# Sara-H-dev/Semantic_Segmentation_Of_StyleGAN2_Artifacts

Hardware: AMD Instinct MI355X
Metric: training images/sec at 1024^2 bs=8 per GPU (MS-UNet Swin-T, fwd+DynamicLoss+bwd+AdamW) (higher is better)
Workload: dtype bf16; 1 GPU; 1xMI355X 1024x1024 bs=8 Swin-T MS-UNet train step; model=MS-UNet swin_t, global_batch=8, world_size=1, img_size=1024, parallelism=dp1, grad_allreduce=f32, dead_branches=executed (no grad), step_execution=eager, params=42881040

## Files before the change

include/msunet_hip.h:

```cpp
#ifndef MSUNET_HIP_H
#define MSUNET_HIP_H

#ifdef __cplusplus
extern "C" {
#endif

int msu_layernorm_fwd(int dtype, int mode, const void* x, const void* b, const float* bscale,
                      long rows_per_sample, void* s_out, const float* gamma, const float* beta,
                      void* y, float* mean, float* rstd, long rows, int C, int H, int W, int Cin,
                      float eps, void* stream);
int msu_layernorm_bwd(int dtype, int mode, const void* dy, const void* x, const void* dres,
                      const float* gamma, const float* mean, const float* rstd, void* dx,
                      void* db, const float* bscale, long rows_per_sample, float* part,
                      int nparts, float* dgamma, float* dbeta, long rows, int C, int H, int W,
                      int Cin, int accumulate, void* stream);
int msu_layernorm_bwd3(int dtype, int mode, const void* dy, const void* x, const void* dres,
                       const void* dres2, const void* dres3, const float* gamma, const float* mean,
                       const float* rstd, void* dx, void* db, const float* bscale, long rows_per_sample,
                       float* part, int nparts, float* dgamma, float* dbeta, long rows, int C, int H, int W,
                       int Cin, int accumulate, void* stream);
int msu_ln_part_blocks(long rows, int C);
int msu_colsum_batch(int nseg, const float* const* part, const long* stride, const int* nparts, const int* n,
                     float* const* out, int accumulate, void* stream);
int msu_tail_reduce_mode(int mode);
// ... 27 lines not shown
                     void* stream);
int msu_win_attn_bwd2(int dtype, const void* qkv, const float* qkv_bias, const float* table,
                      const void* dout, void* dqkv, float* dtable, float* dqkv_bias_pad,
                      float* workspace, int B, int H, int W, int C, int nh, int shift,
                      float p_drop, unsigned long long seed, const unsigned long long* seed_dev, const void* keep,
                      void* stream, void* param_stream);
int msu_win_attn_bwd_tail(int dtype, float* workspace, float* dtable, float* dqkv_bias_pad, int B, int H, int W,
                          int C, int nh, void* stream);
int msu_win_attn_bwd_tail2(int dtype, float* workspace, float* dtable, float* dqkv_bias_pad, int B, int H, int W,
                           int C, int nh, int accumulate, void* stream);

int msu_conv3x3_fwd(int dtype, int in_mode, const void* X, const void* Wt, const float* bias,
                    void* Y, int B, int H, int W, int Cin, int Cout, void* stream);
int msu_conv3x3_fwd2(int dtype, int in_mode, const void* X, const void* Wt, const float* bias,
                     void* Y, void* Y2, int B, int H, int W, int Cin, int Cout, void* stream);
int msu_conv3x3_dgrad(int dtype, int out_mode, const void* dY, const void* Wflip, const void* S,
                      void* dX, int B, int H, int W, int Cin, int Cout, void* stream);
int msu_conv_mode(int mode);
long msu_conv3x3_wgrad_workspace(int nchunk, int Cin, int Cout, int dtype, int unused);
int msu_conv3x3_wgrad(int dtype, int in_mode, const void* X, const void* dY, float* dW, float* db,
                      float* workspace, void* unused, int nchunk, int B, int H, int W, int Cin,
                      int Cout, void* stream);
int msu_conv3x3_wgrad2(int dtype, int in_mode, const void* X, const void* dY, float* dW, float* db,
                       float* workspace, int nchunk, int B, int H, int W, int Cin, int Cout, int accumulate,
                       void* stream);

int msu_win_attn_qkv_supported(int C, int nh);
int msu_win_attn_qkv_fwd(int dtype, const void* x, const void* w_qkv, const float* b_qkv, const float* table,
                         void* out, void* qkv_out, void* keep, float* workspace, int B, int H, int W, int C, int nh,
                         int shift, float p_drop, unsigned long long seed, const unsigned long long* seed_dev,
// ... 99 lines not shown
```

semantic_segmentation_of_stylegan2_artifacts_amd/_lib.py:

```python
import ctypes
import os

from . import switches

_HERE = os.path.dirname(os.path.abspath(__file__))
LIB_PATH = switches.get("MSU_LIB_OVERRIDE") or os.path.join(_HERE, "libmsunet_hip.so")

P = ctypes.c_void_p
I = ctypes.c_int
L = ctypes.c_long
F = ctypes.c_float
D = ctypes.c_double
U64 = ctypes.c_ulonglong

SIGNATURES = {
    "msu_ln_part_blocks": (I, [L, I]),
    "msu_layernorm_fwd": (I, [I, I, P, P, P, L, P, P, P, P, P, P, L, I, I, I, I, F, P]),
    "msu_layernorm_bwd": (I, [I, I, P, P, P, P, P, P, P, P, P, L, P, I, P, P, L, I, I, I, I, I, P]),
    "msu_layernorm_bwd3": (I, [I, I, P, P, P, P, P, P, P, P, P, P, P, L, P, I, P, P, L, I, I, I, I, I, P]),
    "msu_reduce_rows": (I, [P, I, I, L, P, I, P]),
    "msu_tail_reduce_mode": (I, [I]),
    "msu_conv_mode": (I, [I]),
    "msu_head_fwd": (I, [I, P, P, P, P, P, P, P, L, I, F, P]),
    "msu_head_bwd": (I, [I, P, P, P, P, P, P, P, P, P, I, P, P, P, L, I, P]),
# ... 23 lines not shown
    "msu_dynloss_fwd2": (I, [I, P, P, I, L, F, F, F, P, I, P, P, P, P]),
    "msu_dynloss_fwd3": (I, [I, P, P, I, L, F, F, F, P, I, P, P, P, P, P]),
    "msu_dynloss_bwd2": (I, [I, P, P, P, P, P, I, L, F, F, F, P, P]),
    "msu_adamw": (I, [P, P, P, P, L, F, F, F, F, F, I, P, P, P]),
    "msu_nonfinite": (I, [P, L, P, P]),
    "msu_nonfinite2": (I, [P, L, P, L, P, P]),
    "msu_adamw_dev": (I, [P, P, P, P, L, P, D, D, D, D, P, P, P]),
    "msu_adamw_dev2": (I, [P, P, P, P, L, P, D, D, D, D, P, P, P, I, I, P]),
    "msu_step_advance": (I, [P, P, P]),
    "msu_cast": (I, [I, P, P, L, P]),
    "msu_colsum_batch": (I, [I, P, P, P, P, P, I, P]),
    "msu_conv3x3_weight": (I, [I, P, P, I, I, I, P]),
    "msu_transpose16_multi": (I, [P, P, P, I, I, P]),
    "msu_conv3x3_fwd": (I, [I, I, P, P, P, P, I, I, I, I, I, P]),
    "msu_conv3x3_fwd2": (I, [I, I, P, P, P, P, P, I, I, I, I, I, P]),
    "msu_conv3x3_dgrad": (I, [I, I, P, P, P, P, I, I, I, I, I, P]),
    "msu_conv3x3_wgrad_workspace": (L, [I, I, I, I, I]),
    "msu_conv3x3_wgrad": (I, [I, I, P, P, P, P, P, P, I, I, I, I, I, I, P]),
    "msu_conv3x3_wgrad2": (I, [I, I, P, P, P, P, P, I, I, I, I, I, I, I, P]),
    "msu_wgrad_splits": (I, [L, I, I]),
    "msu_wgrad_workspace": (L, [L, I, I]),
    "msu_linear_wgrad": (I, [I, P, P, P, P, P, L, I, I, I, P]),
    "msu_linear_wgrad_ld": (I, [I, P, P, P, L, P, P, L, I, I, I, P]),
    "msu_linear_bwd_supported": (I, [L, I, I]),
    "msu_linear_bwd_workspace": (L, [L, I, I]),
    "msu_linear_bwd": (I, [I, P, P, P, P, P, P, P, P, L, I, I, I, P]),
    "msu_tok_gemm_supported": (I, [L, I, I]),
    "msu_tok_gemm_supported_epi": (I, [L, I, I, I]),
    "msu_tok_gemm": (I, [I, P, P, I, P, P, P, P, P, L, I, I, I, P]),
    "msu_tok_gemm_plan": (I, [L, I, I, P]),
# ... 13 lines not shown
_lib = None


class HipLibraryError(RuntimeError):
    pass


def lib():
    global _lib
    if _lib is not None:
        return _lib
    if not os.path.exists(LIB_PATH):
        raise HipLibraryError(
            f"{LIB_PATH} not found: build it with "
            "`python -m semantic_segmentation_of_stylegan2_artifacts_amd.build` (no CPU fallback)")
    h = ctypes.CDLL(LIB_PATH)
    for name, (res, args) in SIGNATURES.items():
        fn = getattr(h, name)
        fn.restype = res
        fn.argtypes = args
    h.msu_nt_gemm_mode((1 if switches.on("MSU_NT_PP") else 0) | (16 if switches.on("MSU_NT_DYN") else 0))
    h.msu_tail_reduce_mode(1 if switches.on("MSU_TAIL") else 0)
    h.msu_conv_mode(1 if switches.on("MSU_CONV_DYN") else 0)
    _lib = h
    return _lib


def plan_nt(M, N):
    v = lib().msu_nt_gemm_plan(M, N)
    return (v % 1000000) // 1000, v % 1000, v >= 1000000


def call(name, *args):
    rc = getattr(lib(), name)(*args)
    if rc != 0:
        raise HipLibraryError(f"{name} failed with code {rc}")
# ... 2 lines not shown
```

semantic_segmentation_of_stylegan2_artifacts_amd/csrc/conv3x3.h:

```cpp
#pragma once
#include <cstdlib>
#include <utility>

#include "common.h"
#include "mfma_frag.h"
#include "reduce.h"

#ifndef MSU_EXP
#define MSU_EXP 0
#endif

namespace {

constexpr int TW = 16;

struct ConvGeom {
  int B, H, W;
  int Cin, CinP;
  int Cout;
  int PS;
  int PSW;
  int PSD;
};

// ... 423 lines not shown
          }
        }
    }
  }
}

constexpr int V3_HALO_TAP = 1;
constexpr int SPRE = 12;
constexpr bool SP_AT7 = (MSU_EXP & 1024) != 0;

MSU_DEV int swz(int p) { return (p >> 2) & 3; }
template <bool M16> MSU_DEV int swzv(int p) { return M16 ? (p >> 1) & 3 : (p >> 2) & 3; }

MSU_DEV constexpr int halo_part_lo(int t, int nhc) { return (t - 1) * nhc / 7; }

template <typename T, bool IN_D2S, bool OUT_D2S, bool OUT_GGRAD, bool BIAS, bool DUAL, bool SPREAD, bool M16>
__global__ void __launch_bounds__(512) conv3x3_v3_kernel(const bf16_t* __restrict__ X,
                                                         const bf16_t* __restrict__ Wt,
                                                         const float* __restrict__ bias,
                                                         const bf16_t* __restrict__ S,
                                                         bf16_t* __restrict__ Y, bf16_t* __restrict__ Y2,
                                                         ConvGeom g, int ntiles, int* __restrict__ tq) {
  constexpr int C = 96, CH = 12, NW = 8, MT = 2, TH = NW * MT, TWV = 32, HWD = TWV + 2;
  constexpr int HPIX = (TH + 2) * HWD;
  (void)HPIX;
  constexpr int NTHR = 64 * NW;
  constexpr int PSTEP = NTHR / CH;
  constexpr int NHC = (HPIX + PSTEP - 1) / PSTEP;
  constexpr int WIMG = C * C;
  constexpr int WINS = WIMG * 2 / 1024;
  constexpr int WPER = (WINS + NW - 1) / NW;
  static_assert(WINS * 1024 == WIMG * 2, "weight image in whole DMA instructions");

  extern __shared__ __attribute__((aligned(16))) unsigned char smem_raw[];
  bf16_t* sX = reinterpret_cast<bf16_t*>(smem_raw);
  bf16_t* sW = sX + HPIX * C;
  float* sB = reinterpret_cast<float*>(sW + 2 * WIMG);
  int* sQ = reinterpret_cast<int*>(sB + C);
  const int tid = threadIdx.x, lane = tid & 63;
  const int wave = __builtin_amdgcn_readfirstlane(tid >> 6);
  const int tiles_x = (g.W + TWV - 1) / TWV, tiles_y = (g.H + TH - 1) / TH;
  constexpr int EST = MT * 6 * (DUAL ? 2 : 1);
  const int per_img = tiles_x * tiles_y;

  auto coords = [&](int tile, int& b, int& y0, int& x0) {
    b = tile / per_img;
    const int r = tile - b * per_img;
    y0 = (r / tiles_x) * TH;
    x0 = (r - (r / tiles_x) * tiles_x) * TWV;
  };
  u32x4 hr[NHC];
  auto load_halo = [&](int tile, auto C0, auto C1) {
    constexpr int c0 = decltype(C0)::value, c1 = decltype(C1)::value;
    int b, y0, x0;
    coords(tile, b, y0, x0);
    const int t = opaque(tid);
    const bool hact = t < PSTEP * CH;
// ... 48 lines not shown

  auto finish = [&]() { tq_finish(tq); };
  auto read_q = [&]() -> int {
    uint32_t v = ds_b32_untracked<0>(lds_u32(sQ));
    lds_wait_tie<0>(v);
    return __builtin_amdgcn_readfirstlane((int)v) + (int)gridDim.x;
  };
  int tile = blockIdx.x;
  if (tile >= ntiles) {
    finish();
    return;
  }
  if (tq != nullptr && tid == 0) sQ[0] = tq_claim(tq, 0);
  if constexpr (BIAS) {
    if (tid < C) sB[tid] = bias[tid];
  }
  load_halo(tile, IC<0>{}, IC<NHC>{});
  store_halo();
  dma_w(0, 0);
  __syncthreads();
  int next = tq != nullptr ? read_q() : tile + (int)gridDim.x;
  int wbuf = 0;
  bool w1_early = false, st_full = false;

  const int xl = lane & 31, h = lane >> 5;
  auto koff = [&](int sw, int odd) { return ((2 * odd + h) ^ sw) << 3; };
  const int wsw = swz(xl);
  const int wk0 = xl * C + koff(wsw, 0), wk1 = xl * C + koff(wsw, 1);
  const int l15 = lane & 15, g4 = lane >> 4;
  const int wk16 = l15 * C + ((g4 ^ swzv<true>(l15)) << 3);
// ... 203 lines not shown
      }
      wbuf ^= 1;
    }, std::make_integer_sequence<int, 9>{});
    auto epi_start = [&]() __attribute__((always_inline)) {
      if constexpr (OUT_GGRAD) {
        wait_vmcnt<0>();
#pragma unroll
        for (int m = 0; m < MT; ++m)
#pragma unroll
          for (int n = 0; n < (M16 ? 2 : 3); ++n)
#pragma unroll
            for (int pp = 0; pp < (M16 ? 3 : 2); ++pp) vreg_pin(sp[m][n][pp]);
      }
      w1_early = next < ntiles;
      st_full = w1_early && x0 + TWV <= g.W && y0 + TH <= g.H;
      if (w1_early) dma_w(1, wbuf ^ 1);
    };

    if constexpr (M16) {
      const int cofs = 16 * (g4 & 1) + 8 * (g4 >> 1);
      float4 bq[3][2];
      if constexpr (BIAS) {
#pragma unroll
        for (int q = 0; q < 3; ++q) {
          bq[q][0] = *reinterpret_cast<const float4*>(sB + 32 * q + cofs);
          bq[q][1] = *reinterpret_cast<const float4*>(sB + 32 * q + cofs + 4);
        }
      }
      epi_start();
#pragma unroll
      for (int pt = 0; pt < 2; ++pt) {
        const int px = x0 + 16 * pt + l15;
        if (px >= g.W) continue;
#pragma unroll
        for (int q = 0; q < 3; ++q) {
          float bv[8] = {0.f, 0.f, 0.f, 0.f, 0.f, 0.f, 0.f, 0.f};
          if constexpr (BIAS) {
            const float4 t0 = bq[q][0], t1 = bq[q][1];
            bv[0] = t0.x; bv[1] = t0.y; bv[2] = t0.z; bv[3] = t0.w;
            bv[4] = t1.x; bv[5] = t1.y; bv[6] = t1.z; bv[7] = t1.w;
          }
#pragma unroll
          for (int m = 0; m < MT; ++m) {
            const int y = y0 + 2 * wave + m;
// ... 9 lines not shown
            if constexpr (OUT_GGRAD) {
              const u32x4 t = sp[m][pt][q];
#pragma unroll
              for (int i = 0; i < 4; ++i) {
                v[2 * i] *= gelu_grad_fast(Fmt16<T>::lo(t[i]));
                v[2 * i + 1] *= gelu_grad_fast(Fmt16<T>::hi(t[i]));
              }
            }
            const u32x4 pk = {pack2<T>(v[0], v[1]), pack2<T>(v[2], v[3]), pack2<T>(v[4], v[5]), pack2<T>(v[6], v[7])};
            const int off = pix_off32<OUT_D2S>(b, y, px, g.H, g.W, C) + 32 * q + cofs;
            if constexpr (MSU_EXP & 64) if (v[0] != 1.2345e-30f) continue;
            *reinterpret_cast<u32x4*>(Y + off) = pk;
            if constexpr (DUAL) *reinterpret_cast<u32x4*>(Y2 + off) = gelu8<T>(pk);
          }
        }
      }
    } else {
    float4 bq[3][2][2];
    if constexpr (BIAS) {
#pragma unroll
      for (int n = 0; n < 3; ++n)
#pragma unroll
        for (int pp = 0; pp < 2; ++pp) {
          const int co = 32 * n + 16 * pp + 8 * h;
          bq[n][pp][0] = *reinterpret_cast<const float4*>(sB + co);
          bq[n][pp][1] = *reinterpret_cast<const float4*>(sB + co + 4);
        }
    }
    epi_start();
    if (xo < g.W) {
// ... 369 lines not shown
  static_assert(lds <= 160 * 1024, "LDS");
  auto kern = conv3x3_v2_kernel<T, NCT, KS, NW, MT, WDB, IN_D2S, IN_GELU, OUT_D2S, OUT_GGRAD, BIAS, DUAL>;
  static bool attr_set = false;
  if (!attr_set) {
    (void)hipFuncSetAttribute((const void*)kern, hipFuncAttributeMaxDynamicSharedMemorySize, (int)lds);
    attr_set = true;
  }
  const long ntiles = (long)g.B * ((g.W + 31) / 32) * ((g.H + TH - 1) / TH);
  if (ntiles == 0) return 0;
  if ((long)g.B * g.H * g.W * (g.Cin > g.Cout ? g.Cin : g.Cout) >= (1L << 31)) return -2;
  const int grid = (int)(ntiles < num_cus() ? ntiles : num_cus());
  hipLaunchKernelGGL(kern, dim3(grid), dim3(64 * NW), lds, st, X, Wt, bias, S, Y, Y2, g, (int)ntiles);
  return MSU_CHECK_LAUNCH();
}

template <typename T, bool IN_D2S, bool OUT_D2S, bool OUT_GGRAD, bool BIAS, bool DUAL, bool SPREAD, bool M16>
int launch_v3s(const ConvGeom& g, const bf16_t* X, const bf16_t* Wt, const float* bias, const bf16_t* S, bf16_t* Y,
               bf16_t* Y2, hipStream_t st) {
  constexpr size_t lds = sizeof(bf16_t) * ((size_t)18 * 34 * 96 + 2 * 96 * 96) + 96 * sizeof(float) + 16;
  static_assert(lds <= 160 * 1024, "LDS");
  auto kern = conv3x3_v3_kernel<T, IN_D2S, OUT_D2S, OUT_GGRAD, BIAS, DUAL, SPREAD, M16>;
  static bool attr_set = false;
  if (!attr_set) {
    (void)hipFuncSetAttribute((const void*)kern, hipFuncAttributeMaxDynamicSharedMemorySize, (int)lds);
    attr_set = true;
  }
  const long ntiles = (long)g.B * ((g.W + 31) / 32) * ((g.H + 15) / 16);
  if (ntiles == 0) return 0;
  if ((long)g.B * g.H * g.W * 96 >= (1L << 31)) return -2;
  const int grid = (int)(ntiles < num_cus() ? ntiles : num_cus());
  hipLaunchKernelGGL(kern, dim3(grid), dim3(512), lds, st, X, Wt, bias, S, Y, Y2, g, (int)ntiles,
                     g_conv_dyn ? tile_queue(st) : nullptr);
  return MSU_CHECK_LAUNCH();
}

template <typename T, bool IN_D2S, bool OUT_D2S, bool OUT_GGRAD, bool BIAS, bool DUAL>
int launch_v3(const ConvGeom& g, const bf16_t* X, const bf16_t* Wt, const float* bias, const bf16_t* S, bf16_t* Y,
              bf16_t* Y2, hipStream_t st) {
  if constexpr (!OUT_GGRAD || (MSU_EXP & 2048) != 0)
    return launch_v3s<T, IN_D2S, OUT_D2S, OUT_GGRAD, BIAS, DUAL, true, true>(g, X, Wt, bias, S, Y, Y2, st);
  return launch_v3s<T, IN_D2S, OUT_D2S, OUT_GGRAD, BIAS, DUAL, true, false>(g, X, Wt, bias, S, Y, Y2, st);
}

template <typename T, bool IN_D2S, bool IN_GELU, bool OUT_D2S, bool OUT_GGRAD, bool BIAS, bool DUAL = false>
int conv_nt(const ConvGeom& g, const void* X, const void* Wt, const float* bias, const void* S,
            void* Y, void* Y2, hipStream_t st) {
  const T* x = (const T*)X; const T* w = (const T*)Wt; const T* s = (const T*)S; T* y = (T*)Y; T* y2 = (T*)Y2;
  if constexpr (sizeof(T) == 2 && !IN_GELU) {
// ... 76 lines not shown
```

semantic_segmentation_of_stylegan2_artifacts_amd/csrc/conv3x3.hip:

```cpp
#include "conv3x3.h"

extern "C" {

int msu_conv3x3_fwd2(int dtype, int in_mode, const void* X, const void* Wt, const float* bias,
                     void* Y, void* Y2, int B, int H, int W, int Cin, int Cout, void* stream) {
  if (Cout % 16 || Cin % 8 || Cout > 128 || Cin > 128) return -2;
  if ((in_mode & 2) && (H % 4 || W % 4)) return -2;
  if (Y2 && (in_mode & 1)) return -2;
  const ConvGeom g = make_geom(B, H, W, Cin, Cout, msu_is16(dtype) ? 2 : 4);
  hipStream_t st = (hipStream_t)stream;
  if (bias == nullptr) return -2;
#define MSU_FWD(T, D2S, GL, DU) return conv_nt<T, D2S, GL, false, false, true, DU>(g, X, Wt, bias, nullptr, Y, Y2, st)
#define MSU_FWD_ALL(T)                              \
  switch ((in_mode & 3) | (Y2 ? 4 : 0)) {           \
    case 0: MSU_FWD(T, false, false, false);        \
    case 1: MSU_FWD(T, false, true, false);         \
    case 2: MSU_FWD(T, true, false, false);         \
    case 3: MSU_FWD(T, true, true, false);          \
    case 4: MSU_FWD(T, false, false, true);         \
    case 6: MSU_FWD(T, true, false, true);          \
  }
  if (dtype == MSU_BF16) {
    MSU_FWD_ALL(bf16_t)
  } else if (dtype == MSU_F16) {
    MSU_FWD_ALL(f16_t)
  } else {
    MSU_FWD_ALL(float)
  }
#undef MSU_FWD_ALL
#undef MSU_FWD
  return -3;
}

int msu_conv3x3_fwd(int dtype, int in_mode, const void* X, const void* Wt, const float* bias,
                    void* Y, int B, int H, int W, int Cin, int Cout, void* stream) {
  return msu_conv3x3_fwd2(dtype, in_mode, X, Wt, bias, Y, nullptr, B, H, W, Cin, Cout, stream);
}

int msu_conv3x3_dgrad(int dtype, int out_mode, const void* dY, const void* Wflip, const void* S,
                      void* dX, int B, int H, int W, int Cin, int Cout, void* stream) {
  if (Cout % 16 || Cin % 16 || Cout > 128 || Cin > 128) return -2;
  if ((out_mode & 2) && (H % 4 || W % 4)) return -2;
  const ConvGeom g = make_geom(B, H, W, Cout, Cin, msu_is16(dtype) ? 2 : 4);
  hipStream_t st = (hipStream_t)stream;
#define MSU_DG(T, D2S, GG) return conv_nt<T, false, false, D2S, GG, false>(g, dY, Wflip, nullptr, S, dX, nullptr, st)
  if (dtype == MSU_BF16) {
    switch (out_mode & 3) {
      case 1: MSU_DG(bf16_t, false, true);
      case 3: MSU_DG(bf16_t, true, true);
    }
  } else if (dtype == MSU_F16) {
    switch (out_mode & 3) {
      case 1: MSU_DG(f16_t, false, true);
// ... 20 lines not shown
```

semantic_segmentation_of_stylegan2_artifacts_amd/network/model_parts.py:

```python
import math
import random

import torch
import torch.nn as nn
import torch.nn.functional as F

from .. import ops


def _trunc_normal_(t, std=0.02):
    return nn.init.trunc_normal_(t, std=std)


def _to_2tuple(v):
    return tuple(v) if isinstance(v, (tuple, list)) else (v, v)


def _relative_position_index(ws):
    coords = torch.stack(torch.meshgrid(torch.arange(ws), torch.arange(ws), indexing="ij"))
    flat = coords.flatten(1)
    rel = (flat[:, :, None] - flat[:, None, :]).permute(1, 2, 0).contiguous()
    rel[:, :, 0] += ws - 1
    rel[:, :, 1] += ws - 1
    rel[:, :, 0] *= 2 * ws - 1
# ... 289 lines not shown

    def __init__(self, input_resolution, dim, dim_scale=4, norm_layer=nn.LayerNorm):
        super().__init__()
        self.input_resolution = input_resolution
        self.dim = dim
        self.dim_scale = dim_scale
        if dim_scale != 4:
            raise ValueError("FinalPatchExpand_X4_V2 is a x4 expand")
        self.expand = nn.Linear(dim, 16 * dim, bias=False)
        self.act = nn.GELU()
        self.output_dim = dim
        self.refine1 = nn.Conv2d(dim, dim, kernel_size=3, padding=1, bias=True)
        self.refine2 = nn.Conv2d(dim, dim, kernel_size=3, padding=1, bias=True)
        self.norm = norm_layer(self.output_dim)

    def pre_norm(self, x):
        H, W = self.input_resolution
        B, L, C = x.shape
        assert L == H * W, "input feature has wrong size"
        e, a0 = ops.linear_gelu(x, self.expand.weight)
        e, a0 = e.view(B, H, W, 16 * C), a0.view(B, H, W, 16 * C)
        z1, a1 = ops.refine_conv_act(e, a0, self.refine1.weight, self.refine1.bias, True, (4 * H, 4 * W), dual=True)
        return ops.refine_conv_act(z1, a1, self.refine2.weight, self.refine2.bias, False, (4 * H, 4 * W))

    def forward(self, x):
        z2 = self.pre_norm(x)
        B = z2.shape[0]
        y = ops.layer_norm(z2, self.norm.weight, self.norm.bias, self.norm.eps)
        return y.reshape(B, -1, self.output_dim)


class BasicLayer_up(nn.Module):

    def __init__(self, dim, input_resolution, depth, num_heads, window_size, mlp_ratio=4.0,
                 qkv_bias=True, qk_scale=None, drop=0.0, attn_drop=0.0, drop_path=0.0,
                 norm_layer=nn.LayerNorm, upsample=None, use_checkpoint=False):
        super().__init__()
        self.dim = dim
# ... 192 lines not shown
            else:
                x = _skip_fuse(self.concat_back_dim[k], x, xd[3 - k], keys[3 - k] if keys else 0)
                x = layer_up(x)
        return ops.layer_norm(x, self.norm_up.weight, self.norm_up.bias, self.norm_up.eps)

    def up_x4(self, x):
        H, W = self.patches_resolution
        if x.dim() == 4:
            B, H, W, C = x.shape
            x = x.reshape(B, H * W, C)
        else:
            B, L, C = x.shape
            assert L == H * W, "input features has wrong size"
        if self.final_upsample != "expand_first":
            return x
        z2 = self.up.pre_norm(x)
        if self.num_classes == 1:
            return ops.head_norm_output(z2, self.up.norm.weight, self.up.norm.bias, self.output.weight,
                                        self.up.norm.eps)
        y = ops.layer_norm(z2, self.up.norm.weight, self.up.norm.bias, self.up.norm.eps)
        return ops.linear(y, self.output.weight.reshape(self.num_classes, -1)).permute(0, 3, 1, 2)

    def forward(self, x):
        x, xd, xk = self._forward_features(x)
        x = self.forward_up_features(x, xd, xk)
        return self.up_x4(x)

    def freeze_encoder(self, freeze=True):
        for p in self.patch_embed.parameters():
            p.requires_grad = not freeze
# ... 16 lines not shown
```

semantic_segmentation_of_stylegan2_artifacts_amd/ops.py:

```python
import contextlib
import ctypes
import functools

import torch

from . import _lib, switches

_DT = {torch.float32: 0, torch.bfloat16: 1, torch.float16: 2}
_LOW = (torch.bfloat16, torch.float16)


def _dt(t):
    try:
        return _DT[t.dtype]
    except KeyError:
        raise TypeError(f"unsupported activation dtype {t.dtype} (float32 / bfloat16 / float16)") from None


def _need_cuda(*ts):
    for t in ts:
        if t is not None and not t.is_cuda:
            raise RuntimeError("msunet HIP ops need tensors on a HIP device (no CPU fallback)")


# ... 1301 lines not shown

def _head_fake(z, gamma, beta, w, eps):
    B, H, W, C = z.shape
    rows = B * H * W
    return (z.new_empty(B, 1, H, W, dtype=torch.float32), z.new_empty(rows, dtype=torch.float32),
            z.new_empty(rows, dtype=torch.float32))


def _head_setup(ctx, inputs, output):
    z, gamma, beta, w, eps = inputs
    ctx.save_for_backward(z.contiguous(), gamma, beta, w, output[1], output[2])
    ctx.params = (gamma, beta, w)
    ctx.set_materialize_grads(False)


def _head_backward(ctx, dlogit, _dm, _dr):
    z, gamma, beta, w, mean, rstd = ctx.saved_tensors
    if dlogit is None:
        return None, None, None, None, None
    B, H, W, C = z.shape
    rows = B * H * W
    dlogit = _f32(dlogit)
    dz = torch.empty_like(z)
    direct = _direct(*ctx.params)
    if direct:
        dg, db, dw = (p.grad for p in ctx.params)
    else:
        dg, db, dw = torch.empty(3, C, device=z.device, dtype=torch.float32)
    n, part = _ln_parts(rows, C, z.device)
    _lib.call("msu_head_bwd2", _dt(z), _p(dlogit), _p(z), _p(gamma), _p(beta), _p(w), _p(mean),
              _p(rstd), _p(dz), _p(part), n, _p(dg), _p(db), _p(dw), rows, C, int(direct), _s(z))
    if direct:
        _notify(*ctx.params)
        return dz, None, None, None, None
    return dz, dg, db, dw.view(w.shape), None


_head = _define("head_norm_output",
                "(Tensor z, Tensor gamma, Tensor beta, Tensor w, float eps) -> (Tensor, Tensor, Tensor)",
                _head_impl, _head_fake, _head_setup, _head_backward)


def head_norm_output(z, gamma, beta, out_weight, eps=1e-5):
    if out_weight.shape[0] != 1:
        raise ValueError("fused head supports num_classes == 1")
    w = _f32(out_weight).contiguous()
    return _head(_as(z, act_dtype()), _f32(gamma), _f32(beta), w, float(eps))[0]


_CONV_WGRAD_BLOCKS = int(switches.get("MSU_CONV_WGRAD_BLOCKS"))
# ... 96 lines not shown

def _refine_act_fake(x, a, weight, bias, d2s, H, W, dual):
    z = a.new_empty(a.shape[0], H, W, weight.shape[0])
    return z, (torch.empty_like(z) if dual else z.new_empty(0))


def _refine_act_setup(ctx, inputs, output):
    x, a, weight, bias, d2s, H, W, dual = inputs
    ctx.save_for_backward(x, a.contiguous(), weight)
    ctx.params = (weight, bias)
    ctx.cfg = (d2s, H, W)
    ctx.mark_non_differentiable(output[1])
    ctx.set_materialize_grads(False)


def _refine_act_backward(ctx, dz, _dz2):
    x, a, weight = ctx.saved_tensors
    d2s, H, W = ctx.cfg
    if dz is None:
        return (None,) * 8
    Cout, Cin = weight.shape[0], weight.shape[1]
    B = a.shape[0]
    dz = _as(dz, a.dtype)
    dx = None
    if ctx.needs_input_grad[0]:
        wf = _conv_weight(weight, a.dtype, 1)
        dx = torch.empty_like(x)
        _lib.call("msu_conv3x3_dgrad", _dt(a), 1 | (2 if d2s else 0), _p(dz), _p(wf), _p(x), _p(dx),
                  B, H, W, Cin, Cout, _s(a))
    dw, db = _conv_wgrad_param(a, dz, 2 if d2s else 0, B, H, W, Cin, Cout, *ctx.params)
    return dx, None, dw, db, None, None, None, None


_refine_conv_act = _define(
    "refine_conv_act",
    "(Tensor x, Tensor a, Tensor weight, Tensor bias, bool d2s, int H, int W, bool dual) -> (Tensor, Tensor)",
    _refine_act_impl, _refine_act_fake, _refine_act_setup, _refine_act_backward)


def refine_conv_act(x, a, weight, bias, d2s, out_hw, dual=False):
    dt = act_dtype()
    H, W = out_hw
    z, z2 = _refine_conv_act(_as(x, dt), _as(a, dt), _f32(weight), _f32(bias), bool(d2s), int(H), int(W),
                             bool(dual))
    return (z, z2) if dual else z


_zero_bias_cache = {}


def _zero_bias(N, device):
    key = (N, str(device))
    z = _zero_bias_cache.get(key)
    if z is None:
        z = torch.zeros(N, device=device, dtype=torch.float32)
        if not torch.cuda.is_current_stream_capturing():
            _zero_bias_cache[key] = z
    return z


# ... 253 lines not shown
```

semantic_segmentation_of_stylegan2_artifacts_amd/switches.py:

```python
import os
import warnings

SWITCHES = {
    "MSU_LIB_OVERRIDE": ("", "path of another libmsunet_hip.so (tools/build_exp.sh ablation builds)",
                         "DESIGN 4c"),
    "MSU_WGRAD_SIDE": ("1", "0: every weight gradient on the main stream (determinism bisection)",
                       "DESIGN 4b, 7 (side stream +1.6 %)"),
    "MSU_ATTN_QKV": ("1", "0: the unfused stage-0 qkv Linear + window attention + proj",
                     "DESIGN 4d (r04c: +0.8 %)"),
    "MSU_GEMM_ROUTE": ("", "force a GEMM route: lib (hipBLASLt) / tok / nt",
                       "DESIGN 7 (r03c: hand-written +2.7 % over hipBLASLt)"),
    "MSU_NT_PP": ("0", "1: the ping-pong NT GEMM (gemm_pp.h) where it tiles exactly, else the persistent one",
                  "DESIGN 7 (r05g: 0.72-0.98x of the persistent kernel; no-store ablation 1.07-1.66x)"),
    "MSU_LINBWD": ("1", "0: stage-0 Linear backward as input-gradient GEMM + side-stream weight gradient",
                   "DESIGN 7 (r03af: one-pass +1.4 %)"),
    "MSU_CONV_SIDE": ("1", "0: the refine-conv weight gradients on the main stream",
                      "DESIGN 7 (r04s: side +0.2 %)"),
    "MSU_TAIL": ("1", "0: LayerNorm parameter-gradient partials summed by a colsum launch, not in the kernel",
                 "DESIGN 7 (r05i: +0.5 %, host -4 ms/step)"),
    "MSU_ATTN_AUX": ("1", "0: each attention backward rebuilds its relative-bias image instead of reusing the "
                     "forward's workspace", "DESIGN 7 (r05az)"),
    "MSU_MLP_INFER": ("1", "0: no-grad stage-0 MLPs on the token-GEMM pair instead of the fused kernel",
                      "DESIGN 7 (r05am: +1.3 %)"),
    "MSU_MLP_LN": ("1", "0: no-grad stage-0 blocks run norm2's residual-add LayerNorm as its own kernel before the "
                   "fused MLP", "DESIGN 7 (r05at)"),
    "MSU_MLP_TRAIN": ("1", "0: training stage-0 MLPs on the token-GEMM pair (H and GELU(H) stored) instead of "
                      "the fused kernel storing H only", "DESIGN 7 (r05ao)"),
    "MSU_LN_DEFER": ("1", "0: each LayerNorm backward sums its parameter-gradient partials itself (in-kernel "
                     "tail) instead of one batched reduction per width", "DESIGN 7 (r06)"),
    "MSU_NT_DYN": ("0", "1: the NT GEMM's two-stage kernel claims tiles from a per-XCD device queue (measured "
                   "-0.3 % step, 1.8 % slower standalone: r06q/r06r)", "DESIGN 7 (r06)"),
    "MSU_CONV_DYN": ("1", "0: the refine-conv kernel's static tile schedule (blockIdx.x + k * gridDim.x) instead "
                     "of the device tile queue", "DESIGN 7 (r06)"),
    "MSU_CONV_WGRAD_BLOCKS": ("256", "persistent workgroups of the refine-conv weight gradient (one per CU by "
                              "default; fewer leave CUs to the main stream)", "DESIGN 7 (r04ac, r06)"),
    "MSU_MLP_S1": ("1", "0: the stage-1 training MLPs on the GEMM pair (H and GELU(H) stored) instead of the "
                   "fused kernel streaming its weights through an LDS ring", "DESIGN 7 (r06)"),
    "MSU_RES_HANDOFF": ("1", "0: a stage's first Swin block sums its input's two gradients (norm1 LayerNorm, norm2 "
                        "residual) with an ATen add instead of inside the LayerNorm backward", "DESIGN 7 (r06)"),
    "MSU_GRAPH": ("auto", "HIP-graph replay of the step: 1 / 0 / auto (replay when launch-bound)",
                  "DESIGN 4b (512^2: 401 vs 249-307 img/s)"),
    "MSU_GRAPH_SIDE": ("0", "1: fork the side stream into the captured graph (nondeterministic on ROCm 7.2)",
                       "DESIGN 4b (r03h)"),
}

VALUES = {name: os.environ.get(name, d[0]) for name, d in SWITCHES.items()}


def get(name):
    return VALUES[name]


def on(name):
    return VALUES[name] != "0"
# ... 15 lines not shown
```

Before: 178.8 images/s.

## Fuse decoder head LayerNorm and 1x1 output conv into refine2 conv epilogue

Adds a HEAD variant of the refine conv kernel whose epilogue computes the per-pixel LayerNorm statistics and the dot product with gamma*w_out, writing the logit, mean and rstd directly. When gradients are needed it still stores z for the backward pass. This removes the separate head forward kernel and its re-read of the full-resolution 96-channel activation. It also removes the unused NT_DYN switch. The cost is a longer epilogue with extra cross-lane reductions and more register pressure in the conv kernel.

Measured after the change: 179.5 images/s, median of 6. No clear change (+0.4%).

```diff
diff --git a/include/msunet_hip.h b/include/msunet_hip.h
--- a/include/msunet_hip.h
+++ b/include/msunet_hip.h
@@ -65,6 +65,10 @@
                     void* Y, int B, int H, int W, int Cin, int Cout, void* stream);
 int msu_conv3x3_fwd2(int dtype, int in_mode, const void* X, const void* Wt, const float* bias,
                      void* Y, void* Y2, int B, int H, int W, int Cin, int Cout, void* stream);
+int msu_conv3x3_fwd_head(int dtype, int mode, const void* A, const void* Wt, const float* bias, void* Z,
+                         const float* gamma, const float* beta, const float* w_out, float* logit,
+                         float* mean, float* rstd, int B, int H, int W, int Cin, int Cout, float eps,
+                         void* stream);
 int msu_conv3x3_dgrad(int dtype, int out_mode, const void* dY, const void* Wflip, const void* S,
                       void* dX, int B, int H, int W, int Cin, int Cout, void* stream);
 int msu_conv_mode(int mode);
diff --git a/semantic_segmentation_of_stylegan2_artifacts_amd/_lib.py b/semantic_segmentation_of_stylegan2_artifacts_amd/_lib.py
--- a/semantic_segmentation_of_stylegan2_artifacts_amd/_lib.py
+++ b/semantic_segmentation_of_stylegan2_artifacts_amd/_lib.py
@@ -61,6 +61,7 @@
     "msu_transpose16_multi": (I, [P, P, P, I, I, P]),
     "msu_conv3x3_fwd": (I, [I, I, P, P, P, P, I, I, I, I, I, P]),
     "msu_conv3x3_fwd2": (I, [I, I, P, P, P, P, P, I, I, I, I, I, P]),
+    "msu_conv3x3_fwd_head": (I, [I, I, P, P, P, P, P, P, P, P, P, P, I, I, I, I, I, F, P]),
     "msu_conv3x3_dgrad": (I, [I, I, P, P, P, P, I, I, I, I, I, P]),
     "msu_conv3x3_wgrad_workspace": (L, [I, I, I, I, I]),
     "msu_conv3x3_wgrad": (I, [I, I, P, P, P, P, P, P, I, I, I, I, I, I, P]),
@@ -104,12 +105,13 @@
         raise HipLibraryError(
             f"{LIB_PATH} not found: build it with "
             "`python -m semantic_segmentation_of_stylegan2_artifacts_amd.build` (no CPU fallback)")
+    import torch
     h = ctypes.CDLL(LIB_PATH)
     for name, (res, args) in SIGNATURES.items():
         fn = getattr(h, name)
         fn.restype = res
         fn.argtypes = args
-    h.msu_nt_gemm_mode((1 if switches.on("MSU_NT_PP") else 0) | (16 if switches.on("MSU_NT_DYN") else 0))
+    h.msu_nt_gemm_mode(1 if switches.on("MSU_NT_PP") else 0)
     h.msu_tail_reduce_mode(1 if switches.on("MSU_TAIL") else 0)
     h.msu_conv_mode(1 if switches.on("MSU_CONV_DYN") else 0)
     _lib = h
diff --git a/semantic_segmentation_of_stylegan2_artifacts_amd/csrc/conv3x3.h b/semantic_segmentation_of_stylegan2_artifacts_amd/csrc/conv3x3.h
--- a/semantic_segmentation_of_stylegan2_artifacts_amd/csrc/conv3x3.h
+++ b/semantic_segmentation_of_stylegan2_artifacts_amd/csrc/conv3x3.h
@@ -461,13 +461,40 @@
 
 MSU_DEV constexpr int halo_part_lo(int t, int nhc) { return (t - 1) * nhc / 7; }
 
-template <typename T, bool IN_D2S, bool OUT_D2S, bool OUT_GGRAD, bool BIAS, bool DUAL, bool SPREAD, bool M16>
+struct ConvHead {
+  const float* gamma;
+  const float* beta;
+  const float* w;
+  float* logit;
+  float* mean;
+  float* rstd;
+  float eps;
+};
+
+MSU_DEV float quad_sum(float s) {
+  auto r = __builtin_amdgcn_permlane16_swap(__float_as_uint(s), __float_as_uint(s), false, false);
+  s = __uint_as_float(r[0]) + __uint_as_float(r[1]);
+  r = __builtin_amdgcn_permlane32_swap(__float_as_uint(s), __float_as_uint(s), false, false);
+  return __uint_as_float(r[0]) + __uint_as_float(r[1]);
+}
+
+template <int OFF>
+MSU_DEV f32x4 ds_b128_untracked(uint32_t addr) {
+  f32x4 v;
+  asm volatile("ds_read_b128 %0, %1 offset:%2" : "=v"(v) : "v"(addr), "i"(OFF));
+  return v;
+}
+
+template <typename T, bool IN_D2S, bool OUT_D2S, bool OUT_GGRAD, bool BIAS, bool DUAL, bool SPREAD, bool M16,
+          bool HEAD = false>
 __global__ void __launch_bounds__(512) conv3x3_v3_kernel(const bf16_t* __restrict__ X,
                                                          const bf16_t* __restrict__ Wt,
                                                          const float* __restrict__ bias,
                                                          const bf16_t* __restrict__ S,
                                                          bf16_t* __restrict__ Y, bf16_t* __restrict__ Y2,
-                                                         ConvGeom g, int ntiles, int* __restrict__ tq) {
+                                                         ConvGeom g, int ntiles, int* __restrict__ tq,
+                                                         ConvHead hd) {
+  static_assert(!HEAD || (M16 && BIAS && !OUT_D2S && !OUT_GGRAD && !DUAL), "HEAD: the refine2 forward form");
   constexpr int C = 96, CH = 12, NW = 8, MT = 2, TH = NW * MT, TWV = 32, HWD = TWV + 2;
   constexpr int HPIX = (TH + 2) * HWD;
   (void)HPIX;
@@ -484,10 +511,11 @@
   bf16_t* sW = sX + HPIX * C;
   float* sB = reinterpret_cast<float*>(sW + 2 * WIMG);
   int* sQ = reinterpret_cast<int*>(sB + C);
+  float* sG = reinterpret_cast<float*>(sQ + 4);
   const int tid = threadIdx.x, lane = tid & 63;
   const int wave = __builtin_amdgcn_readfirstlane(tid >> 6);
   const int tiles_x = (g.W + TWV - 1) / TWV, tiles_y = (g.H + TH - 1) / TH;
-  constexpr int EST = MT * 6 * (DUAL ? 2 : 1);
+  constexpr int EST = MT * 6 * (DUAL ? 2 : 1) + (HEAD ? MT * 2 * 3 : 0);
   const int per_img = tiles_x * tiles_y;
 
   auto coords = [&](int tile, int& b, int& y0, int& x0) {
@@ -566,6 +594,21 @@
   if (tq != nullptr && tid == 0) sQ[0] = tq_claim(tq, 0);
   if constexpr (BIAS) {
     if (tid < C) sB[tid] = bias[tid];
+  }
+  float bwsum = 0.f;
+  if constexpr (HEAD) {
+    if (tid < C) sG[tid] = hd.gamma[tid] * hd.w[tid];
+    float bp[4];
+#pragma unroll
+    for (int l = 0; l < 4; ++l) {
+      bp[l] = 0.f;
+#pragma unroll
+      for (int k = 0; k < 3; ++k)
+#pragma unroll
+        for (int e = 0; e < 8; ++e) bp[l] += hd.beta[(l + 4 * k) * 8 + e] * hd.w[(l + 4 * k) * 8 + e];
+    }
+    bwsum = (bp[0] + bp[2]) + (bp[1] + bp[3]);
+    bwsum = __uint_as_float(__builtin_amdgcn_readfirstlane(__float_as_uint(bwsum)));
   }
   load_halo(tile, IC<0>{}, IC<NHC>{});
   store_halo();
@@ -799,13 +842,16 @@
       }
       w1_early = next < ntiles;
       st_full = w1_early && x0 + TWV <= g.W && y0 + TH <= g.H;
+      if constexpr (HEAD) st_full = st_full && Y != nullptr;
       if (w1_early) dma_w(1, wbuf ^ 1);
     };
 
     if constexpr (M16) {
-      const int cofs = 16 * (g4 & 1) + 8 * (g4 >> 1);
+      const int le = HEAD ? opaque(lane) : lane;
+      const int l15e = le & 15, g4e = le >> 4;
+      const int cofs = 16 * (g4e & 1) + 8 * (g4e >> 1);
       float4 bq[3][2];
-      if constexpr (BIAS) {
+      if constexpr (BIAS && !HEAD) {
 #pragma unroll
         for (int q = 0; q < 3; ++q) {
           bq[q][0] = *reinterpret_cast<const float4*>(sB + 32 * q + cofs);
@@ -813,6 +859,83 @@
         }
       }
       epi_start();
+      if constexpr (HEAD) {
+        const uint32_t ba = lds_u32(sB + cofs), ga = lds_u32(sG + cofs);
+        f32x4 gq[3][2];
+        unroll_for<3>([&](auto Q) {
+          constexpr int q = decltype(Q)::value;
+          gq[q][0] = ds_b128_untracked<4 * 32 * q>(ba);
+          gq[q][1] = ds_b128_untracked<4 * 32 * q + 16>(ba);
+        });
+        lds_wait_tie<0>(gq[0][0], gq[0][1], gq[1][0], gq[1][1], gq[2][0], gq[2][1]);
+        u32x4 pk[2][MT][3];
+        int pix[2][MT];
+        bool in[2][MT];
+#pragma unroll
+        for (int pt = 0; pt < 2; ++pt) {
+          const int px = x0 + 16 * pt + l15e;
+#pragma unroll
+          for (int m = 0; m < MT; ++m) {
+            const int y = y0 + 2 * wave + m;
+            in[pt][m] = px < g.W && y < g.H;
+            pix[pt][m] = (b * g.H + y) * g.W + px;
+#pragma unroll
+            for (int q = 0; q < 3; ++q) {
+              const f32x4 t0 = gq[q][0], t1 = gq[q][1];
+              const float bv[8] = {t0[0], t0[1], t0[2], t0[3], t1[0], t1[1], t1[2], t1[3]};
+              float v[8];
+#pragma unroll
+              for (int i = 0; i < 4; ++i) {
+                const auto r = __builtin_amdgcn_permlane16_swap(__float_as_uint(acc4[m][pt][2 * q][i]),
+                                                                __float_as_uint(acc4[m][pt][2 * q + 1][i]), false, false);
+                v[i] = __uint_as_float(r[0]) + bv[i];
+                v[4 + i] = __uint_as_float(r[1]) + bv[4 + i];
+              }
+              pk[pt][m][q] = u32x4{pack2<T>(v[0], v[1]), pack2<T>(v[2], v[3]), pack2<T>(v[4], v[5]), pack2<T>(v[6], v[7])};
+              if (Y != nullptr && in[pt][m]) *reinterpret_cast<u32x4*>(Y + pix[pt][m] * C + 32 * q + cofs) = pk[pt][m][q];
+            }
+          }
+        }
+        unroll_for<3>([&](auto Q) {
+          constexpr int q = decltype(Q)::value;
+          gq[q][0] = ds_b128_untracked<4 * 32 * q>(ga);
+          gq[q][1] = ds_b128_untracked<4 * 32 * q + 16>(ga);
+        });
+        lds_wait_tie<0>(gq[0][0], gq[0][1], gq[1][0], gq[1][1], gq[2][0], gq[2][1]);
+#pragma unroll
+        for (int pt = 0; pt < 2; ++pt) {
+#pragma unroll
+          for (int m = 0; m < MT; ++m) {
+            float sum = 0.f;
+#pragma unroll
+            for (int q = 0; q < 3; ++q)
+#pragma unroll
+              for (int i = 0; i < 4; ++i) sum += Fmt16<T>::lo(pk[pt][m][q][i]), sum += Fmt16<T>::hi(pk[pt][m][q][i]);
+            const float mu = quad_sum(sum) * (1.0f / C);
+            float var = 0.f, dot = 0.f;
+#pragma unroll
+            for (int q = 0; q < 3; ++q) {
+#pragma unroll
+              for (int i = 0; i < 4; ++i) {
+                const float d0 = Fmt16<T>::lo(pk[pt][m][q][i]) - mu, d1 = Fmt16<T>::hi(pk[pt][m][q][i]) - mu;
+                var += d0 * d0;
+                dot += d0 * gq[q][i >> 1][2 * (i & 1)];
+                var += d1 * d1;
+                dot += d1 * gq[q][i >> 1][2 * (i & 1) + 1];
+              }
+            }
+            const float rs = rsqrtf(quad_sum(var) * (1.0f / C) + hd.eps);
+            dot = quad_sum(dot) * rs + bwsum;
+            if (g4e == 0 && in[pt][m]) {
+              hd.logit[pix[pt][m]] = dot;
+              if (Y != nullptr || hd.mean != nullptr) {
+                hd.mean[pix[pt][m]] = mu;
+                hd.rstd[pix[pt][m]] = rs;
+              }
+            }
+          }
+        }
+      } else {
 #pragma unroll
       for (int pt = 0; pt < 2; ++pt) {
         const int px = x0 + 16 * pt + l15;
@@ -852,6 +975,7 @@
             if constexpr (DUAL) *reinterpret_cast<u32x4*>(Y2 + off) = gelu8<T>(pk);
           }
         }
+      }
       }
     } else {
     float4 bq[3][2][2];
@@ -1251,12 +1375,14 @@
   return MSU_CHECK_LAUNCH();
 }
 
-template <typename T, bool IN_D2S, bool OUT_D2S, bool OUT_GGRAD, bool BIAS, bool DUAL, bool SPREAD, bool M16>
+template <typename T, bool IN_D2S, bool OUT_D2S, bool OUT_GGRAD, bool BIAS, bool DUAL, bool SPREAD, bool M16,
+          bool HEAD = false>
 int launch_v3s(const ConvGeom& g, const bf16_t* X, const bf16_t* Wt, const float* bias, const bf16_t* S, bf16_t* Y,
-               bf16_t* Y2, hipStream_t st) {
-  constexpr size_t lds = sizeof(bf16_t) * ((size_t)18 * 34 * 96 + 2 * 96 * 96) + 96 * sizeof(float) + 16;
+               bf16_t* Y2, hipStream_t st, const ConvHead& hd = ConvHead{}) {
+  constexpr size_t lds = sizeof(bf16_t) * ((size_t)18 * 34 * 96 + 2 * 96 * 96) + 96 * sizeof(float) + 16 +
+                         (HEAD ? 96 * sizeof(float) : 0);
   static_assert(lds <= 160 * 1024, "LDS");
-  auto kern = conv3x3_v3_kernel<T, IN_D2S, OUT_D2S, OUT_GGRAD, BIAS, DUAL, SPREAD, M16>;
+  auto kern = conv3x3_v3_kernel<T, IN_D2S, OUT_D2S, OUT_GGRAD, BIAS, DUAL, SPREAD, M16, HEAD>;
   static bool attr_set = false;
   if (!attr_set) {
     (void)hipFuncSetAttribute((const void*)kern, hipFuncAttributeMaxDynamicSharedMemorySize, (int)lds);
@@ -1267,8 +1393,19 @@
   if ((long)g.B * g.H * g.W * 96 >= (1L << 31)) return -2;
   const int grid = (int)(ntiles < num_cus() ? ntiles : num_cus());
   hipLaunchKernelGGL(kern, dim3(grid), dim3(512), lds, st, X, Wt, bias, S, Y, Y2, g, (int)ntiles,
-                     g_conv_dyn ? tile_queue(st) : nullptr);
+                     g_conv_dyn ? tile_queue(st) : nullptr, hd);
   return MSU_CHECK_LAUNCH();
+}
+
+template <typename T>
+int conv_head(const ConvGeom& g, const void* X, const void* Wt, const float* bias, void* Y, const ConvHead& hd,
+              hipStream_t st) {
+  if constexpr (sizeof(T) == 2) {
+    if (g.Cout == 96 && g.CinP == 96 && g.Cin == 96)
+      return launch_v3s<T, false, false, false, true, false, true, true, true>(
+          g, (const bf16_t*)X, (const bf16_t*)Wt, bias, nullptr, (bf16_t*)Y, nullptr, st, hd);
+  }
+  return -2;
 }
 
 template <typename T, bool IN_D2S, bool OUT_D2S, bool OUT_GGRAD, bool BIAS, bool DUAL>
diff --git a/semantic_segmentation_of_stylegan2_artifacts_amd/csrc/conv3x3.hip b/semantic_segmentation_of_stylegan2_artifacts_amd/csrc/conv3x3.hip
--- a/semantic_segmentation_of_stylegan2_artifacts_amd/csrc/conv3x3.hip
+++ b/semantic_segmentation_of_stylegan2_artifacts_amd/csrc/conv3x3.hip
@@ -37,6 +37,21 @@
   return msu_conv3x3_fwd2(dtype, in_mode, X, Wt, bias, Y, nullptr, B, H, W, Cin, Cout, stream);
 }
 
+int msu_conv3x3_fwd_head(int dtype, int mode, const void* A, const void* Wt, const float* bias, void* Z,
+                         const float* gamma, const float* beta, const float* w_out, float* logit,
+                         float* mean, float* rstd, int B, int H, int W, int Cin, int Cout, float eps,
+                         void* stream) {
+  if (mode != 0 || !msu_is16(dtype) || Cin != 96 || Cout != 96) return -2;
+  if (!bias || !gamma || !beta || !w_out || !logit) return -2;
+  if (Z && (!mean || !rstd)) return -2;
+  if ((mean == nullptr) != (rstd == nullptr)) return -2;
+  const ConvGeom g = make_geom(B, H, W, Cin, Cout, 2);
+  const ConvHead hd{gamma, beta, w_out, logit, mean, rstd, eps};
+  hipStream_t st = (hipStream_t)stream;
+  if (dtype == MSU_BF16) return conv_head<bf16_t>(g, A, Wt, bias, Z, hd, st);
+  return conv_head<f16_t>(g, A, Wt, bias, Z, hd, st);
+}
+
 int msu_conv3x3_dgrad(int dtype, int out_mode, const void* dY, const void* Wflip, const void* S,
                       void* dX, int B, int H, int W, int Cin, int Cout, void* stream) {
   if (Cout % 16 || Cin % 16 || Cout > 128 || Cin > 128) return -2;
diff --git a/semantic_segmentation_of_stylegan2_artifacts_amd/network/model_parts.py b/semantic_segmentation_of_stylegan2_artifacts_amd/network/model_parts.py
--- a/semantic_segmentation_of_stylegan2_artifacts_amd/network/model_parts.py
+++ b/semantic_segmentation_of_stylegan2_artifacts_amd/network/model_parts.py
@@ -327,14 +327,24 @@
         self.refine2 = nn.Conv2d(dim, dim, kernel_size=3, padding=1, bias=True)
         self.norm = norm_layer(self.output_dim)
 
-    def pre_norm(self, x):
+    def pre_refine2(self, x):
         H, W = self.input_resolution
         B, L, C = x.shape
         assert L == H * W, "input feature has wrong size"
         e, a0 = ops.linear_gelu(x, self.expand.weight)
         e, a0 = e.view(B, H, W, 16 * C), a0.view(B, H, W, 16 * C)
-        z1, a1 = ops.refine_conv_act(e, a0, self.refine1.weight, self.refine1.bias, True, (4 * H, 4 * W), dual=True)
+        return ops.refine_conv_act(e, a0, self.refine1.weight, self.refine1.bias, True, (4 * H, 4 * W), dual=True)
+
+    def pre_norm(self, x):
+        H, W = self.input_resolution
+        z1, a1 = self.pre_refine2(x)
         return ops.refine_conv_act(z1, a1, self.refine2.weight, self.refine2.bias, False, (4 * H, 4 * W))
+
+    def head_logits(self, x, out_weight):
+        H, W = self.input_resolution
+        z1, a1 = self.pre_refine2(x)
+        return ops.refine_conv_head(z1, a1, self.refine2.weight, self.refine2.bias, self.norm.weight,
+                                    self.norm.bias, out_weight, self.norm.eps, (4 * H, 4 * W))
 
     def forward(self, x):
         z2 = self.pre_norm(x)
@@ -557,6 +567,8 @@
             assert L == H * W, "input features has wrong size"
         if self.final_upsample != "expand_first":
             return x
+        if self.num_classes == 1 and ops.refine_head_fused(self.up.refine2.weight):
+            return self.up.head_logits(x, self.output.weight)
         z2 = self.up.pre_norm(x)
         if self.num_classes == 1:
             return ops.head_norm_output(z2, self.up.norm.weight, self.up.norm.bias, self.output.weight,
diff --git a/semantic_segmentation_of_stylegan2_artifacts_amd/ops.py b/semantic_segmentation_of_stylegan2_artifacts_amd/ops.py
--- a/semantic_segmentation_of_stylegan2_artifacts_amd/ops.py
+++ b/semantic_segmentation_of_stylegan2_artifacts_amd/ops.py
@@ -1339,26 +1339,30 @@
     ctx.set_materialize_grads(False)
 
 
-def _head_backward(ctx, dlogit, _dm, _dr):
-    z, gamma, beta, w, mean, rstd = ctx.saved_tensors
-    if dlogit is None:
-        return None, None, None, None, None
+def _head_bwd(z, gamma, beta, w, mean, rstd, dlogit, params):
     B, H, W, C = z.shape
     rows = B * H * W
     dlogit = _f32(dlogit)
     dz = torch.empty_like(z)
-    direct = _direct(*ctx.params)
+    direct = _direct(*params)
     if direct:
-        dg, db, dw = (p.grad for p in ctx.params)
+        dg, db, dw = (p.grad for p in params)
     else:
         dg, db, dw = torch.empty(3, C, device=z.device, dtype=torch.float32)
     n, part = _ln_parts(rows, C, z.device)
     _lib.call("msu_head_bwd2", _dt(z), _p(dlogit), _p(z), _p(gamma), _p(beta), _p(w), _p(mean),
               _p(rstd), _p(dz), _p(part), n, _p(dg), _p(db), _p(dw), rows, C, int(direct), _s(z))
     if direct:
-        _notify(*ctx.params)
-        return dz, None, None, None, None
-    return dz, dg, db, dw.view(w.shape), None
+        _notify(*params)
+        return dz, None, None, None
+    return dz, dg, db, dw.view(w.shape)
+
+
+def _head_backward(ctx, dlogit, _dm, _dr):
+    z, gamma, beta, w, mean, rstd = ctx.saved_tensors
+    if dlogit is None:
+        return None, None, None, None, None
+    return (*_head_bwd(z, gamma, beta, w, mean, rstd, dlogit, ctx.params), None)
 
 
 _head = _define("head_norm_output",
@@ -1485,21 +1489,26 @@
     ctx.set_materialize_grads(False)
 
 
+def _refine_act_bwd(x, a, weight, d2s, H, W, dz, params, need_dx):
+    Cout, Cin = weight.shape[0], weight.shape[1]
+    B = a.shape[0]
+    dz = _as(dz, a.dtype)
+    dx = None
+    if need_dx:
+        wf = _conv_weight(weight, a.dtype, 1)
+        dx = torch.empty_like(x)
+        _lib.call("msu_conv3x3_dgrad", _dt(a), 1 | (2 if d2s else 0), _p(dz), _p(wf), _p(x), _p(dx),
+                  B, H, W, Cin, Cout, _s(a))
+    dw, db = _conv_wgrad_param(a, dz, 2 if d2s else 0, B, H, W, Cin, Cout, *params)
+    return dx, dw, db
+
+
 def _refine_act_backward(ctx, dz, _dz2):
     x, a, weight = ctx.saved_tensors
     d2s, H, W = ctx.cfg
     if dz is None:
         return (None,) * 8
-    Cout, Cin = weight.shape[0], weight.shape[1]
-    B = a.shape[0]
-    dz = _as(dz, a.dtype)
-    dx = None
-    if ctx.needs_input_grad[0]:
-        wf = _conv_weight(weight, a.dtype, 1)
-        dx = torch.empty_like(x)
-        _lib.call("msu_conv3x3_dgrad", _dt(a), 1 | (2 if d2s else 0), _p(dz), _p(wf), _p(x), _p(dx),
-                  B, H, W, Cin, Cout, _s(a))
-    dw, db = _conv_wgrad_param(a, dz, 2 if d2s else 0, B, H, W, Cin, Cout, *ctx.params)
+    dx, dw, db = _refine_act_bwd(x, a, weight, d2s, H, W, dz, ctx.params, ctx.needs_input_grad[0])
     return dx, None, dw, db, None, None, None, None
 
 
@@ -1515,6 +1524,99 @@
     z, z2 = _refine_conv_act(_as(x, dt), _as(a, dt), _f32(weight), _f32(bias), bool(d2s), int(H), int(W),
                              bool(dual))
     return (z, z2) if dual else z
+
+
+_HEAD_FUSE = switches.on("MSU_HEAD_FUSE")
+refine_head_calls = 0
+
+
+def _refine_head_impl(x, a, weight, bias, gamma, beta, w, eps, H, W, keep):
+    global refine_head_calls
+    _need_cuda(x, a)
+    a = a.contiguous()
+    Cout, Cin = weight.shape[0], weight.shape[1]
+    B = a.shape[0]
+    dt = a.dtype
+    rows = B * H * W
+    wt = _conv_weight(weight, dt, 0)
+    logit = torch.empty(B, 1, H, W, device=a.device, dtype=torch.float32)
+    z = torch.empty(B, H, W, Cout, device=a.device, dtype=dt) if keep else None
+    mean, rstd = _stats(a, rows) if keep else (None, None)
+    rc = _lib.lib().msu_conv3x3_fwd_head(_dt(a), 0, _p(a), _p(wt), _p(bias), _p(z), _p(gamma), _p(beta), _p(w),
+                                         _p(logit), _p(mean), _p(rstd), B, H, W, Cin, Cout, eps, _s(a))
+    if rc == 0:
+        refine_head_calls += 1
+    elif rc == -2:
+        if not keep:
+            z = torch.empty(B, H, W, Cout, device=a.device, dtype=dt)
+            mean, rstd = _stats(a, rows)
+        _lib.call("msu_conv3x3_fwd2", _dt(a), 0, _p(a), _p(wt), _p(bias), _p(z), None, B, H, W, Cin, Cout, _s(a))
+        _lib.call("msu_head_fwd", _dt(z), _p(z), _p(gamma), _p(beta), _p(w), _p(logit), _p(mean), _p(rstd),
+                  rows, Cout, eps, _s(z))
+    else:
+        raise _lib.HipLibraryError(f"msu_conv3x3_fwd_head failed with code {rc}")
+    if not keep:
+        return a.new_empty(0), logit, logit.new_empty(0), logit.new_empty(0)
+    return z, logit, mean, rstd
+
+
+def _refine_head_fake(x, a, weight, bias, gamma, beta, w, eps, H, W, keep):
+    B = a.shape[0]
+    rows = B * H * W if keep else 0
+    z = a.new_empty(B, H, W, weight.shape[0]) if keep else a.new_empty(0)
+    return (z, a.new_empty(B, 1, H, W, dtype=torch.float32), a.new_empty(rows, dtype=torch.float32),
+            a.new_empty(rows, dtype=torch.float32))
+
+
+def _refine_head_setup(ctx, inputs, output):
+    x, a, weight, bias, gamma, beta, w, eps, H, W, keep = inputs
+    z, logit, mean, rstd = output
+    ctx.save_for_backward(x, a.contiguous(), weight, z, gamma, beta, w, mean, rstd)
+    ctx.conv_params = (weight, bias)
+    ctx.head_params = (gamma, beta, w)
+    ctx.cfg = (H, W)
+    ctx.mark_non_differentiable(mean, rstd)
+    ctx.set_materialize_grads(False)
+
+
+def _refine_head_backward(ctx, dz_in, dlogit, _dm, _dr):
+    x, a, weight, z, gamma, beta, w, mean, rstd = ctx.saved_tensors
+    H, W = ctx.cfg
+    if dlogit is None and dz_in is None:
+        return (None,) * 11
+    if z.numel() == 0:
+        raise RuntimeError("refine_conv_head: backward through a forward that did not keep z (keep=False)")
+    dz, dg, dbt, dwo = (None,) * 4
+    if dlogit is not None:
+        dz, dg, dbt, dwo = _head_bwd(z, gamma, beta, w, mean, rstd, dlogit, ctx.head_params)
+    if dz_in is not None:
+        dz = _as(dz_in, z.dtype) if dz is None else dz + _as(dz_in, z.dtype)
+    dx, dw, db = _refine_act_bwd(x, a, weight, False, H, W, dz, ctx.conv_params, ctx.needs_input_grad[0])
+    return dx, None, dw, db, dg, dbt, dwo, None, None, None, None
+
+
+_refine_conv_head = _define(
+    "refine_conv_head",
+    "(Tensor x, Tensor a, Tensor weight, Tensor bias, Tensor gamma, Tensor beta, Tensor w_out, float eps, "
+    "int H, int W, bool keep) -> (Tensor, Tensor, Tensor, Tensor)",
+    _refine_head_impl, _refine_head_fake, _refine_head_setup, _refine_head_backward)
+
+
+def refine_head_fused(weight):
+    return bool(_HEAD_FUSE and act_dtype() in _LOW and tuple(weight.shape[:2]) == (96, 96))
+
+
+def refine_conv_head(x, a, weight, bias, gamma, beta, out_weight, eps, out_hw, full=False):
+    if out_weight.shape[0] != 1:
+        raise ValueError("fused head supports num_classes == 1")
+    dt = act_dtype()
+    H, W = out_hw
+    w = _f32(out_weight).contiguous()
+    ts = (x, weight, bias, gamma, beta, out_weight)
+    keep = torch.is_grad_enabled() and any(t.requires_grad for t in ts)
+    out = _refine_conv_head(_as(x, dt), _as(a, dt), _f32(weight), _f32(bias), _f32(gamma), _f32(beta), w,
+                            float(eps), int(H), int(W), bool(keep))
+    return out if full else out[1]
 
 
 _zero_bias_cache = {}
diff --git a/semantic_segmentation_of_stylegan2_artifacts_amd/switches.py b/semantic_segmentation_of_stylegan2_artifacts_amd/switches.py
--- a/semantic_segmentation_of_stylegan2_artifacts_amd/switches.py
+++ b/semantic_segmentation_of_stylegan2_artifacts_amd/switches.py
@@ -28,8 +28,6 @@
                       "the fused kernel storing H only", "DESIGN 7 (r05ao)"),
     "MSU_LN_DEFER": ("1", "0: each LayerNorm backward sums its parameter-gradient partials itself (in-kernel "
                      "tail) instead of one batched reduction per width", "DESIGN 7 (r06)"),
-    "MSU_NT_DYN": ("0", "1: the NT GEMM's two-stage kernel claims tiles from a per-XCD device queue (measured "
-                   "-0.3 % step, 1.8 % slower standalone: r06q/r06r)", "DESIGN 7 (r06)"),
     "MSU_CONV_DYN": ("1", "0: the refine-conv kernel's static tile schedule (blockIdx.x + k * gridDim.x) instead "
                      "of the device tile queue", "DESIGN 7 (r06)"),
     "MSU_CONV_WGRAD_BLOCKS": ("256", "persistent workgroups of the refine-conv weight gradient (one per CU by "
@@ -38,6 +36,8 @@
                    "fused kernel streaming its weights through an LDS ring", "DESIGN 7 (r06)"),
     "MSU_RES_HANDOFF": ("1", "0: a stage's first Swin block sums its input's two gradients (norm1 LayerNorm, norm2 "
                         "residual) with an ATen add instead of inside the LayerNorm backward", "DESIGN 7 (r06)"),
+    "MSU_HEAD_FUSE": ("1", "0: refine2 and the decoder head (LayerNorm + 1x1 output conv) as two launches instead "
+                      "of the head in refine2's conv epilogue", "DESIGN 7 (r07)"),
     "MSU_GRAPH": ("auto", "HIP-graph replay of the step: 1 / 0 / auto (replay when launch-bound)",
                   "DESIGN 4b (512^2: 401 vs 249-307 img/s)"),
     "MSU_GRAPH_SIDE": ("0", "1: fork the side stream into the captured graph (nondeterministic on ROCm 7.2)",
```
